# Illumina/canvas

Hardware: AMD Instinct MI355X
Metric: genome-bins/sec (bin+clean+partition) (higher is better)
Workload: dtype u8/int32 (bin), f32/f64 (clean, viterbi); 1 GPU; BASELINE configs[2]: whole-genome GRCh38 60x single sample, full bin+clean+partition HIP path on 1 MI355X per sample; bins_after_clean=4686240, bin_size=534, partition=PerSampleHMM, clean_flags=-g -s -r --local-sd-metric-file, segments=250, samples=1

## Files before the change

### canvas_amd/csrc/bin.hip

```cpp
#include "common.hpp"
#include <algorithm>
#include <thread>
#include <emmintrin.h>

#define TILE_SHIFT 12
#define TILE 4096

struct BinChrom {
    const uint8_t* bases;
    const uint8_t* hits;
    const uint64_t* mask;
    int64_t len;
    int64_t tileBase;
    int64_t ntiles;
};

__device__ __forceinline__ int find_chrom(const BinChrom* __restrict__ ch, int nchr, int64_t gtile) {
    int lo = 0, hi = nchr - 1;
    while (lo < hi) {
        int mid = (lo + hi + 1) >> 1;
        if (ch[mid].tileBase <= gtile) lo = mid; else hi = mid - 1;
    }
    return lo;
}
// ... 779 lines not shown
        ProfScope ps(ctx, "gcw_read_gc", false, sp);
        if (rg3) hipLaunchKernelGGL((k_read_gc3<RG3_HE, RG3_HO>), dim3((unsigned)std::min<int64_t>(gridRg, ntileAll)), dim3(256), ldsRg, sp, dRg, nchr, ntileAll, meanFrag, mean40, nWmax, hist);
        else for (int c = 0; c < nchr; c++) {
            const int64_t ntile = (h_len[c] + RG_T - 1) / RG_T;
            hipLaunchKernelGGL(k_read_gc2, dim3((unsigned)std::min<int64_t>(gridRg, ntile)), dim3(256), ldsRg, sp, d_bases[c], d_fraglen[c], d_hits[c], h_len[c], meanFrag, mean40, nWmax,
                               (uint8_t*)gch[c].readGc, hist);
        }
    }
    CANVAS_HIP_TRY(ctx, hipMemcpyAsync(ctx->side_pin, hist, (size_t)RG_REP_ALL * 202 * 8, hipMemcpyDeviceToHost, sp));
    CANVAS_HIP_TRY(ctx, hipEventRecord(ctx->side_ev2, sp));
    P.pending = true;
    if (!P.overlap) { rc0 = gcw_prepass_finish(ctx, P); if (rc0) return rc0; }
    return CANVAS_OK;
}

static int32_t bin_genome_impl(canvas_ctx* ctx, int32_t nchr, const uint8_t* const* d_bases, const uint64_t* const* d_mask,
                               const uint8_t* const* d_hits, const int16_t* const* d_fraglen, const int64_t* h_len, const uint8_t* h_is_auto, int32_t counts_per_bin, int32_t bin_size, int32_t mode,
                               int32_t* d_chr, int32_t* d_start, int32_t* d_stop, int32_t* d_gc, float* d_count, int64_t cap,
                               int32_t* h_bin_size_out, int64_t* h_nbins_per_chr, int64_t* h_nbins_total, cvx_bin_size_hook hook = nullptr, void* hookUser = nullptr,
                               const int64_t* h_pos0_packed = nullptr) {
    if (!ctx) return CANVAS_ERR_INVALID;
    const bool needRates = bin_size <= 0;
    const bool packed = h_pos0_packed != nullptr;
    if (nchr <= 0 || !d_bases || !d_mask || !d_hits || !h_len || (needRates && !hook && (!h_is_auto || counts_per_bin <= 0))) CANVAS_FAIL(ctx, CANVAS_ERR_INVALID, "canvas_bin_genome: bad arguments");
    const bool gcw = mode == CANVAS_MODE_GC_CONTENT_WEIGHTED;
    if (gcw && !d_fraglen) CANVAS_FAIL(ctx, CANVAS_ERR_INVALID, "GCContentWeighted mode needs the fragment-length arrays (canvas_bin_sample_gcweighted)");
    if (gcw && packed) CANVAS_FAIL(ctx, CANVAS_ERR_INVALID, "the packed planes serve Binary and TruncatedDynamicRange; GCContentWeighted reads the per-base arrays");
    if (mode != CANVAS_MODE_BINARY && mode != CANVAS_MODE_TRUNCATED_DYNAMIC_RANGE && !gcw) CANVAS_FAIL(ctx, CANVAS_ERR_INVALID, "unknown coverage mode");
    for (int c = 0; c < nchr; c++) if (h_len[c] <= 0 || h_len[c] > 0x7FFFFFFFll) CANVAS_FAIL(ctx, CANVAS_ERR_INVALID, "chromosome length must be in [1, 2^31)");
    CANVAS_HIP_TRY(ctx, hipSetDevice(ctx->device));
    BinPlan plan = make_plan(nchr, d_bases, d_mask, d_hits, h_len);
    GcwPre gp;
    if (gcw) { ctx->gcw_stats_dev = nullptr; ctx->gcw_total = 0; }
    if (gcw && ctx->up_active) {
        CANVAS_HIP_TRY(ctx, hipStreamSynchronize(ctx->copy)); ctx->up_active = false;
    }
    if (gcw) {
        for (int c = 0; c < nchr; c++) if (((uintptr_t)d_fraglen[c] | (uintptr_t)d_bases[c] | (uintptr_t)d_hits[c]) & 15) CANVAS_FAIL(ctx, CANVAS_ERR_INVALID, "GCContentWeighted mode: bases, hits and fragment lengths must be 16-byte aligned");
        int32_t rc0 = gcw_prepass_begin(ctx, nchr, d_bases, d_hits, d_fraglen, h_len, true, gp); if (rc0) return rc0;
    }
    const int64_t ub = cap;
    WsSizer sz;
    const size_t tabSlots = (size_t)nchr + ((size_t)nchr + sizeof(BinChrom) - 1) / sizeof(BinChrom);
    sz.take<BinChrom>(tabSlots); sz.take<unsigned long long>(nchr); sz.take<uint32_t>(plan.ntiles); sz.take<uint32_t>(plan.ntiles); sz.take<int32_t>(plan.ntiles);
    sz.take<ChromOut>(nchr); sz.take<long long>(nchr + 1); sz.take<uint32_t>(plan.ntiles); sz.take<uint32_t>(plan.ntiles);
    sz.take<int32_t>(ub + 1); sz.take<uint32_t>(ub + 1); sz.take<uint32_t>(ub + 1);
    bool streamed = ctx->up_active && (int)ctx->up_bases.size() == nchr && !gcw;
    for (int c = 0; streamed && c < nchr; c++) streamed = ctx->up_bases[c] == d_bases[c] && ctx->up_mask[c] == d_mask[c] && ctx->up_hits[c] == d_hits[c];
    if (ctx->up_active && !streamed) { CANVAS_HIP_TRY(ctx, hipStreamSynchronize(ctx->copy)); }
    ctx->up_active = false;
    const bool singleRead = packed || streamed || (needRates && !cvx_hook("CANVAS_BIN_TWO_PASS")) || cvx_hook("CANVAS_BIN_SINGLE_READ");
    const int nchunks = (int)((plan.ntiles + TS_CHUNK - 1) / TS_CHUNK);
    if (singleRead) { sz.take<uint32_t>(plan.ntiles * 64); sz.take<uint32_t>(plan.ntiles + 8); sz.take<TsPart>(nchunks + 1); sz.take<TsPart>(nchunks + 1); sz.take<unsigned long long>(nchr);
                      sz.take<TsPart>(nchr + 1); sz.take<ChromDev>(nchr); sz.take<uint4>(ub + 1); }
    int32_t rc = canvas_ws_reserve(ctx, sz.off + 4096); if (rc) return rc;
    const size_t oAuto = (size_t)nchr * sizeof(BinChrom), oOut = (oAuto + (size_t)nchr + 15) & ~size_t(15), oP0 = oOut + (size_t)nchr * sizeof(ChromOut), oBd = oP0 + (size_t)nchr * 8;
    rc = canvas_pin_reserve(ctx, oBd + sizeof(BinDev) + 64); if (rc) return rc;
    WsCarver ws(ctx->ws);
    BinChrom* dCh = ws.take<BinChrom>(tabSlots); unsigned long long* dPos0 = ws.take<unsigned long long>(nchr);
    uint32_t* tilePop = ws.take<uint32_t>(plan.ntiles); uint32_t* tileObs = ws.take<uint32_t>(plan.ntiles); int32_t* rankBase = ws.take<int32_t>(plan.ntiles);
    ChromOut* dOut = ws.take<ChromOut>(nchr); long long* binOffset = ws.take<long long>(nchr + 1);
    uint32_t* tileTotC = ws.take<uint32_t>(plan.ntiles); uint32_t* tileTotG = ws.take<uint32_t>(plan.ntiles);
    int32_t* stopTmp = ws.take<int32_t>(ub + 1); uint32_t* locC = ws.take<uint32_t>(ub + 1); uint32_t* locG = ws.take<uint32_t>(ub + 1);
    uint32_t* wordSum = singleRead ? ws.take<uint32_t>(plan.ntiles * 64) : nullptr;
    uint32_t* rankRaw = nullptr; TsPart* tsPart = nullptr; TsPart* tsPartEx = nullptr; unsigned long long* dPopBefore = nullptr; TsPart* chrPre = nullptr; ChromDev* chrDev = nullptr; uint4* binRec = nullptr; uint8_t* dIsAuto = (uint8_t*)(dCh + nchr);
    if (singleRead) { rankRaw = ws.take<uint32_t>(plan.ntiles + 8); tsPart = ws.take<TsPart>(nchunks + 1); tsPartEx = ws.take<TsPart>(nchunks + 1); dPopBefore = ws.take<unsigned long long>(nchr);
                      chrPre = ws.take<TsPart>(nchr + 1); chrDev = ws.take<ChromDev>(nchr); binRec = ws.take<uint4>(ub + 1); }
    if (singleRead && !ctx->bin_dev) {
        CANVAS_HIP_TRY(ctx, hipMalloc(&ctx->bin_dev, 256)); CANVAS_HIP_TRY(ctx, hipMemsetAsync(ctx->bin_dev, 0, 256, ctx->stream));
        CANVAS_HIP_TRY(ctx, hipEventCreateWithFlags(&ctx->bin_ev, hipEventDisableTiming));
    }
    uint32_t* dTick = (uint32_t*)ctx->bin_dev; BinDev* dBd = (BinDev*)((char*)ctx->bin_dev + 64);
    const int clampHits = mode == CANVAS_MODE_TRUNCATED_DYNAMIC_RANGE ? 1 : 0;
    const bool byVal = nchr <= BIN_BYVAL;
    if (byVal) {
        BinChromPack pack; memset(&pack, 0, sizeof pack);
        memcpy(pack.c, plan.chroms.data(), nchr * sizeof(BinChrom));
        for (int c = 0; c < nchr; c++) {
            pack.isAuto[c] = h_is_auto ? (h_is_auto[c] ? 1 : 0) : 0;
            if (packed) { if (h_pos0_packed[c] < 0 || h_pos0_packed[c] > h_len[c]) CANVAS_FAIL(ctx, CANVAS_ERR_INVALID, "canvas_bin_sample_packed: pos0 outside [0, len]"); pack.pos0[c] = (unsigned long long)h_pos0_packed[c]; }
        }
        hipLaunchKernelGGL(k_bin_begin, dim3(1), dim3(256), 0, ctx->stream, dCh, dIsAuto, pack, nchr, dPos0, packed ? 1 : 0);
    } else {
        memcpy(ctx->pin, plan.chroms.data(), nchr * sizeof(BinChrom));
        for (int c = 0; c < nchr; c++) ((uint8_t*)ctx->pin)[oAuto + c] = h_is_auto ? (h_is_auto[c] ? 1 : 0) : 0;
        CANVAS_HIP_TRY(ctx, hipMemcpyAsync(dCh, ctx->pin, oAuto + (size_t)nchr, hipMemcpyHostToDevice, ctx->stream));
    }
    ChromOut* hOut = (ChromOut*)((char*)ctx->pin + oOut);
    const unsigned pkGrid = (unsigned)((plan.ntiles + 4 * PK_TILES - 1) / (4 * PK_TILES));
    if (packed) {
        if (!byVal) {
            unsigned long long* hp0 = (unsigned long long*)((char*)ctx->pin + oP0);
            for (int c = 0; c < nchr; c++) {
                if (h_pos0_packed[c] < 0 || h_pos0_packed[c] > h_len[c]) CANVAS_FAIL(ctx, CANVAS_ERR_INVALID, "canvas_bin_sample_packed: pos0 outside [0, len]");
                hp0[c] = (unsigned long long)h_pos0_packed[c];
            }
            CANVAS_HIP_TRY(ctx, hipMemcpyAsync(dPos0, hp0, (size_t)nchr * 8, hipMemcpyHostToDevice, ctx->stream));
        }
        if (streamed) {
            for (int c = 0; c < nchr; c++) {
                const BinChrom& C = plan.chroms[c];
                CANVAS_HIP_TRY(ctx, hipStreamWaitEvent(ctx->stream, ctx->up_ev[c], 0));
                ProfScope ps(ctx, "bin_summary_packed_streamed", true);
                hipLaunchKernelGGL(k_tile_summary_packed, dim3((unsigned)((C.ntiles + 4 * PK_TILES - 1) / (4 * PK_TILES))), dim3(256), 0, ctx->stream, dCh, nchr, C.tileBase + C.ntiles, dPos0,
                                   clampHits, needRates ? 1 : 0, wordSum, tilePop, tileObs, tileTotC, tileTotG, C.tileBase);
            }
        } else {
            ProfScope ps(ctx, "bin_summary_packed", true);
            hipLaunchKernelGGL(k_tile_summary_packed, dim3(pkGrid), dim3(256), 0, ctx->stream, dCh, nchr, plan.ntiles, dPos0, clampHits, needRates ? 1 : 0,
                               wordSum, tilePop, tileObs, tileTotC, tileTotG, (int64_t)0);
        }
    } else {
    if (!byVal) hipLaunchKernelGGL(k_init_pos0, dim3((nchr + 63) / 64), dim3(64), 0, ctx->stream, dCh, nchr, dPos0);
    if (streamed) {
        for (int c = 0; c < nchr; c++) {
            const BinChrom& C = plan.chroms[c];
            CANVAS_HIP_TRY(ctx, hipStreamWaitEvent(ctx->stream, ctx->up_ev[c], 0));
            hipLaunchKernelGGL(k_find_pos0, dim3(64, 1), dim3(256), 0, ctx->stream, dCh, dPos0, c);
            ProfScope ps(ctx, "bin_summary_streamed", true);
            hipLaunchKernelGGL(k_tile_summary, dim3((unsigned)((C.ntiles + 3) / 4)), dim3(256), 0, ctx->stream, dCh, nchr, C.tileBase + C.ntiles, dPos0, clampHits, needRates ? 1 : 0,
                               wordSum, tilePop, tileObs, tileTotC, tileTotG, C.tileBase);
            hipLaunchKernelGGL(k_tile_summary_edges, dim3(2), dim3(64), 0, ctx->stream, dCh, nchr, dPos0, clampHits, needRates ? 1 : 0, wordSum, tilePop, tileObs, tileTotC, tileTotG, c);
        }
    } else hipLaunchKernelGGL(k_find_pos0, dim3(64, nchr), dim3(256), 0, ctx->stream, dCh, dPos0, 0);
    if (streamed) {
    } else if (singleRead) {
        ProfScope ps(ctx, "bin_summary", true);
        hipLaunchKernelGGL(k_tile_summary, dim3((unsigned)((plan.ntiles + 3) / 4)), dim3(256), 0, ctx->stream, dCh, nchr, plan.ntiles, dPos0, clampHits, needRates ? 1 : 0,
                           wordSum, tilePop, tileObs, tileTotC, tileTotG, (int64_t)0);
    } else {
        ProfScope ps(ctx, "bin_tile_stats", true);
        hipLaunchKernelGGL(k_tile_stats, dim3((unsigned)((plan.ntiles + 3) / 4)), dim3(256), 0, ctx->stream, dCh, nchr, plan.ntiles, needRates ? 1 : 0, tilePop, tileObs);
    }
    if (singleRead && !streamed) hipLaunchKernelGGL(k_tile_summary_edges, dim3(2 * nchr), dim3(64), 0, ctx->stream, dCh, nchr, dPos0, clampHits, needRates ? 1 : 0, wordSum, tilePop, tileObs, tileTotC, tileTotG, 0);
    }
    int64_t total = 0;
    if (singleRead) {
        const int binSizeArg = !needRates ? bin_size : (hook ? -1 : 0);
        const uint32_t* obsArr = needRates ? tileObs : (const uint32_t*)nullptr;
        unsigned* hBdSeq = (unsigned*)((char*)ctx->pin + oBd + sizeof(BinDev));
        const unsigned bdSeq = hook ? 0u : cvx_mail_arm(ctx, hBdSeq);
        hipLaunchKernelGGL(k_tscan_reduce, dim3((unsigned)(nchunks + nchr)), dim3(TS_T), 0, ctx->stream, dCh, nchr, dPos0, packed ? 1 : 0, plan.ntiles, nchunks, tilePop, obsArr, tileTotC, tileTotG,
                           tsPart, tsPartEx, dPopBefore, dTick);
        hipLaunchKernelGGL(k_tscan_apply, dim3((unsigned)nchunks), dim3(TS_T), 0, ctx->stream, dCh, nchr, plan.ntiles, nchunks, tilePop, obsArr, tileTotC, tileTotG, rankRaw, tsPartEx, dPopBefore, chrPre,
                           dIsAuto, counts_per_bin, binSizeArg, (long long)cap, dOut, chrDev, binOffset, dBd, dTick + 1, hook ? (ChromOut*)nullptr : hOut, hook ? (BinDev*)nullptr : (BinDev*)((char*)ctx->pin + oBd),
                           hBdSeq, bdSeq);
        auto launch_close_resolve = [&]() {
            { ProfScope ps(ctx, "bin_close");
              hipLaunchKernelGGL(k_bin_close2, dim3((unsigned)((plan.ntiles + 4 * CLOSE_TILES - 1) / (4 * CLOSE_TILES))), dim3(256), 0, ctx->stream, dCh, chrDev, nchr, plan.ntiles, wordSum, rankRaw,
                                 tileTotC, tileTotG, binOffset, dBd, binRec, d_chr); }
            ProfScope ps(ctx, "bin_resolve");
            static const unsigned gridP = resident_grid((const void*)k_bin_resolve_fin<true>, 256, ctx->device), gridB = resident_grid((const void*)k_bin_resolve_fin<false>, 256, ctx->device);
            if (packed) hipLaunchKernelGGL((k_bin_resolve_fin<true>), dim3(gridP), dim3(256), 0, ctx->stream, dCh, chrDev, binOffset, dPos0, dBd, clampHits, binRec, d_start, d_stop, d_gc, d_count);
            else hipLaunchKernelGGL((k_bin_resolve_fin<false>), dim3(gridB), dim3(256), 0, ctx->stream, dCh, chrDev, binOffset, dPos0, dBd, clampHits, binRec, d_start, d_stop, d_gc, d_count);
        };
        auto host_totals = [&]() {
            total = 0;
            for (int c = 0; c < nchr; c++) { hOut[c].nbins = (hOut[c].pop - hOut[c].popBefore) / bin_size; if (h_nbins_per_chr) h_nbins_per_chr[c] = hOut[c].nbins; total += hOut[c].nbins; }
        };
        if (hook) {
            CANVAS_HIP_TRY(ctx, hipMemcpyAsync(hOut, dOut, nchr * sizeof(ChromOut), hipMemcpyDeviceToHost, ctx->stream));
            CANVAS_HIP_TRY(ctx, hipStreamSynchronize(ctx->stream));
            std::vector<long long> o(nchr), p(nchr), pb(nchr);
            for (int c = 0; c < nchr; c++) { o[c] = hOut[c].obs; p[c] = hOut[c].pop; pb[c] = hOut[c].popBefore; }
            int32_t rch = hook(hookUser, nchr, o.data(), p.data(), pb.data(), &bin_size); if (rch) return rch;
            if (bin_size <= 0) CANVAS_FAIL(ctx, CANVAS_ERR_INVALID, "derived bin size is not positive");
            if (h_bin_size_out) *h_bin_size_out = bin_size;
            host_totals();
            if (h_nbins_total) *h_nbins_total = total;
            if (total > cap) CANVAS_FAIL(ctx, CANVAS_ERR_CAPACITY, "canvas_bin_genome: output capacity too small (see canvas_bin_count_upper_bound)");
            if (total == 0) return CANVAS_OK;
            hipLaunchKernelGGL(k_bin_plan, dim3(1), dim3(TS_T), 0, ctx->stream, nchr, dOut, binOffset, dBd, bin_size, (long long)cap);
            launch_close_resolve();
        } else {
            BinDev* hBd = (BinDev*)((char*)ctx->pin + oBd);
            CANVAS_HIP_TRY(ctx, hipEventRecord(ctx->bin_ev, ctx->stream));
            launch_close_resolve();
            CANVAS_HIP_TRY(ctx, hipEventSynchronize(ctx->bin_ev));
            { int32_t rcm = cvx_mail_await(ctx, hBdSeq, bdSeq, "canvas_bin: bin size and totals"); if (rcm) return rcm; }
            if (needRates && (hBd->flags & (BD_BAD_RATE | BD_TOO_MANY))) {
                std::vector<double> rates;
                for (int c = 0; c < nchr; c++) if (h_is_auto[c]) rates.push_back((int)hOut[c].obs / (double)(int)hOut[c].pop);
                bin_size = canvas_bin_size_from_rates(rates.data(), (int32_t)rates.size(), counts_per_bin);
                if (bin_size <= 0) CANVAS_FAIL(ctx, CANVAS_ERR_INVALID, "derived bin size is not positive");
                host_totals();
                if (total <= cap && total > 0) { hipLaunchKernelGGL(k_bin_plan, dim3(1), dim3(TS_T), 0, ctx->stream, nchr, dOut, binOffset, dBd, bin_size, (long long)cap); launch_close_resolve(); }
            } else {
                if (needRates && (hBd->flags & BD_NO_AUTOSOME)) CANVAS_FAIL(ctx, CANVAS_ERR_INVALID, "no autosome to derive the bin size from");
                bin_size = hBd->binSize;
                if (bin_size <= 0) CANVAS_FAIL(ctx, CANVAS_ERR_INVALID, "derived bin size is not positive");
                total = hBd->total;
                for (int c = 0; c < nchr; c++) if (h_nbins_per_chr) h_nbins_per_chr[c] = hOut[c].nbins;
            }
            if (h_bin_size_out) *h_bin_size_out = bin_size;
            if (h_nbins_total) *h_nbins_total = total;
            if (total > cap) CANVAS_FAIL(ctx, CANVAS_ERR_CAPACITY, "canvas_bin_genome: output capacity too small (see canvas_bin_count_upper_bound)");
            if (total == 0) return CANVAS_OK;
        }
    } else {
    if (needRates) {
        hipLaunchKernelGGL(k_scan_tiles, dim3(nchr), dim3(1024), 0, ctx->stream, dCh, dPos0, tilePop, tileObs, 1, 0, rankBase, dOut, packed ? 1 : 0);
        CANVAS_HIP_TRY(ctx, hipMemcpyAsync(hOut, dOut, nchr * sizeof(ChromOut), hipMemcpyDeviceToHost, ctx->stream));
        CANVAS_HIP_TRY(ctx, hipStreamSynchronize(ctx->stream));
        if (hook) {
            std::vector<long long> o(nchr), p(nchr), pb(nchr);
            for (int c = 0; c < nchr; c++) { o[c] = hOut[c].obs; p[c] = hOut[c].pop; pb[c] = hOut[c].popBefore; }
            int32_t rch = hook(hookUser, nchr, o.data(), p.data(), pb.data(), &bin_size); if (rch) return rch;
// ... 440 lines not shown
```

### canvas_amd/csrc/bin_tail.hpp

```cpp
#pragma once

struct BinDev {
    int32_t binSize;
    int32_t run;
    unsigned long long binMagic;
    long long total;
    int32_t flags;
    int32_t nAuto;
};
#define BD_NO_AUTOSOME 1
#define BD_BAD_RATE 2
#define BD_TOO_MANY 4
#define BD_CAPACITY 8
struct ChromDev { uint32_t rank0, c0, g0, pad; };
struct TsPart { uint32_t pop, obs, c, g; };

#define TS_T 1024
#define TS_ITEMS 8
#define TS_CHUNK (TS_T * TS_ITEMS)
#define BD_MAX_AUTO 2048

template <class T> __device__ __forceinline__ void ts_publish(T* p, T v) { __hip_atomic_store(p, v, __ATOMIC_RELAXED, __HIP_MEMORY_SCOPE_AGENT); }
__device__ __forceinline__ bool ts_arrive_last(uint32_t* tick, uint32_t expected, int* sFlag) {
    asm volatile("s_waitcnt vmcnt(0)" ::: "memory");
// ... 177 lines not shown
            const int item = (int)(rel % TS_ITEMS);
            TsPart o = {0, 0, 0, 0};
#pragma unroll
            for (int i = 0; i < TS_ITEMS; i++) if (i == item) { o.pop = rp[i]; o.obs = ro[i]; o.c = rc[i]; o.g = rg[i]; }
            ts_publish(&chrPre[c].pop, o.pop); ts_publish(&chrPre[c].obs, o.obs); ts_publish(&chrPre[c].c, o.c); ts_publish(&chrPre[c].g, o.g);
        }
    }
    if (!ts_arrive_last(tick, gridDim.x, &sLast)) return;
    const TsPart grand = partEx[nchunks];
    if (tid == 0) { sN = 0; sFlags = 0; sBinSize = binSizeArg > 0 ? binSizeArg : 0; }
    __syncthreads();
    {
        const int per = (nchr + TS_T - 1) / TS_T;
        const int cA = tid * per < nchr ? tid * per : nchr, cB = cA + per < nchr ? cA + per : nchr;
        for (int c = cA; c < cB; c++) {
            const TsPart a = chrPre[c], e = c + 1 < nchr ? chrPre[c + 1] : grand;
            const unsigned long long pb = popBefore[c];
            ChromOut o; o.pop = (long long)(uint32_t)(e.pop - a.pop); o.obs = (long long)(uint32_t)(e.obs - a.obs); o.nbins = 0; o.popBefore = (long long)pb;
            dOut[c] = o;
            ChromDev d; d.rank0 = a.pop + (uint32_t)pb; d.c0 = a.c; d.g0 = a.g; d.pad = 0;
            chrDev[c] = d;
            if (binSizeArg == 0 && isAuto[c]) {
                if (o.pop <= 0) atomicOr(&sFlags, BD_BAD_RATE);
                const int slot = atomicAdd(&sN, 1);
                if (slot < BD_MAX_AUTO) sRate[slot] = (double)(int)o.obs / (double)(int)o.pop;
            }
        }
    }
    __syncthreads();
    if (binSizeArg == 0) {
        const int n = sN;
        if (n == 0) { if (tid == 0) sFlags |= BD_NO_AUTOSOME; }
        else if (n > BD_MAX_AUTO) { if (tid == 0) sFlags |= BD_TOO_MANY; }
        else if (!(sFlags & BD_BAD_RATE)) {
            for (int i = tid; i < n; i += TS_T) {
                const double r = sRate[i]; int rank = 0;
                for (int j = 0; j < n; j++) { const double q = sRate[j]; rank += (q < r || (q == r && j < i)) ? 1 : 0; }
                sSorted[rank] = r;
            }
            __syncthreads();
            if (tid == 0) {
                const double med = (n % 2) ? sSorted[n / 2] : (sSorted[n / 2 - 1] + sSorted[n / 2]) / 2;
                const double q = (double)countsPerBin / med;
                sBinSize = (q >= 1.0 && q < 2147483648.0) ? (int)q : 0;
            }
        }
        __syncthreads();
    }
    if (binSizeArg < 0) return;
    __syncthreads();
    plan_offsets(nchr, dOut, dOut, binOffset, bd, sBinSize, cap, sFlags, sN, sh16, hostOut, hostBd, hostSeq, seq);
}

__global__ void __launch_bounds__(256) k_bin_close2(const BinChrom* __restrict__ ch, const ChromDev* __restrict__ chrDev, int nchr, int64_t ntilesTotal, const uint32_t* __restrict__ S,
                                                    const uint32_t* __restrict__ rankRaw, const uint32_t* __restrict__ tileExC, const uint32_t* __restrict__ tileExG,
                                                    const long long* __restrict__ binOffset, const BinDev* __restrict__ bd,
                                                    uint4* __restrict__ binRec, int32_t* __restrict__ oChr) {
    const int64_t gtile0 = ((int64_t)blockIdx.x * 4 + __builtin_amdgcn_readfirstlane((int)(threadIdx.x >> 6))) * CLOSE_TILES;
    if (gtile0 >= ntilesTotal) return;
    if (!bd->run) return;
    const int binSize = bd->binSize; const unsigned long long binMagic = bd->binMagic;
    const int l = lane_id();
    uint32_t sv[CLOSE_TILES], rk[CLOSE_TILES], tc[CLOSE_TILES], tg[CLOSE_TILES];
#pragma unroll
    for (int t = 0; t < CLOSE_TILES; t++) {
        const bool in = gtile0 + t < ntilesTotal;
        sv[t] = in ? S[(gtile0 + t) * 64 + l] : 0u;
        rk[t] = in ? rankRaw[gtile0 + t] : 0u;
        tc[t] = in ? tileExC[gtile0 + t] : 0u;
        tg[t] = in ? tileExG[gtile0 + t] : 0u;
    }
    int c = find_chrom(ch, nchr, gtile0);
    int64_t tileBase = ch[c].tileBase, tileEnd = tileBase + ch[c].ntiles;
    long long boff = binOffset[c];
    uint32_t rank0 = chrDev[c].rank0;
#pragma unroll
    for (int t = 0; t < CLOSE_TILES; t++) {
        const int64_t gtile = gtile0 + t;
        if (gtile >= ntilesTotal) break;
        while (gtile >= tileEnd) { c++; tileBase = ch[c].tileBase; tileEnd = tileBase + ch[c].ntiles; boff = binOffset[c]; rank0 = chrDev[c].rank0; }
        const uint32_t s = sv[t];
        const uint32_t pop = SUM_POP(s);
        const uint32_t pg = pop | (SUM_GC(s) << 16), cl = SUM_HITS(s);
        const uint32_t pgInc = wave_inclusive_scan_u32(pg), cInc = wave_inclusive_scan_u32(cl);
        const int32_t r = (int32_t)(rk[t] - rank0) + (int32_t)((pgInc - pg) & 0xFFFFu);
        if (pop > 0 && r + (int32_t)pop >= binSize) {
            const uint32_t gEx = tg[t] + ((pgInc - pg) >> 16), cEx = tc[t] + (cInc - cl);
            const int64_t wstart = ((gtile - tileBase) << TILE_SHIFT) + (int64_t)l * 64;
            const int32_t rr = r < 0 ? 0 : r;
            uint32_t q = binMagic ? (uint32_t)__umul64hi((unsigned long long)(uint32_t)rr, binMagic) : (uint32_t)rr;
            uint32_t nextB = (q + 1u) * (uint32_t)binSize;
            for (; (int64_t)nextB - r <= (int64_t)pop && (int64_t)nextB - r >= 1; q++) {
                const long long bin = boff + (long long)q;
                binRec[bin] = make_uint4((uint32_t)(wstart + ((int64_t)nextB - r - 1)), cEx, gEx, (uint32_t)c);
                oChr[bin] = c;
                nextB += (uint32_t)binSize;
            }
        }
    }
}

template <class T> __device__ __forceinline__ uint4 gload_uint4_nt(gptr<T> p) { const canvas_u32x4 v = __builtin_nontemporal_load(reinterpret_cast<gptr<const canvas_u32x4>>(p)); return make_uint4(v.x, v.y, v.z, v.w); }
template <class T> __device__ __forceinline__ ulonglong2 gload_ulonglong2_nt(gptr<T> p) { const canvas_u64x2 v = __builtin_nontemporal_load(reinterpret_cast<gptr<const canvas_u64x2>>(p)); return make_ulonglong2(v.x, v.y); }

__device__ __forceinline__ uint32_t kth_set_bit(uint64_t m, uint32_t kk) {
    uint32_t pos = 0, cnt;
    cnt = __popc((uint32_t)m);           if (kk > cnt) { kk -= cnt; pos += 32; m >>= 32; }
    cnt = __popc((uint32_t)m & 0xFFFFu); if (kk > cnt) { kk -= cnt; pos += 16; m >>= 16; }
    cnt = __popc((uint32_t)m & 0xFFu);   if (kk > cnt) { kk -= cnt; pos += 8; m >>= 8; }
    cnt = __popc((uint32_t)m & 0xFu);    if (kk > cnt) { kk -= cnt; pos += 4; m >>= 4; }
    cnt = __popc((uint32_t)m & 0x3u);    if (kk > cnt) { kk -= cnt; pos += 2; m >>= 2; }
    cnt = (uint32_t)m & 1u;              if (kk > cnt) { pos += 1; }
    return pos;
}
template <bool PACKED>
__global__ void __launch_bounds__(256) k_bin_resolve_fin(const BinChrom* __restrict__ ch, const ChromDev* __restrict__ chrDev, const long long* __restrict__ binOffset,
                                                         const unsigned long long* __restrict__ pos0, const BinDev* __restrict__ bd, int clampHits,
                                                         const uint4* __restrict__ binRec,
                                                         int32_t* __restrict__ oStart, int32_t* __restrict__ oStop, int32_t* __restrict__ oGc, float* __restrict__ oCount) {
    constexpr int LANES = PACKED ? 1 : 4, SLOTS = 256 / LANES, RF_NEW = SLOTS - 1;
    __shared__ int32_t sStop[SLOTS], sChr[SLOTS]; __shared__ uint32_t sC[SLOTS], sG[SLOTS];
    if (!bd->run) return;
    const long long total = bd->total;
    const long long ngroups = (total + RF_NEW - 1) / RF_NEW;
    const int slot = threadIdx.x / LANES, sub = threadIdx.x % LANES;
    for (long long g = blockIdx.x; g < ngroups; g += gridDim.x) {
        const long long i = g * RF_NEW - 1 + slot;
        const bool live = i >= 0 && i < total;
        int32_t stop = 0; uint32_t aC = 0, aG = 0, hc = 0, hg = 0; int c = 0;
        if (live) {
            const uint4 R = binRec[i];
            const int32_t r = (int32_t)R.x;
            c = (int)R.w;
            aC = R.y; aG = R.z;
            const int64_t p0c = (int64_t)pos0[c];
            const int64_t wstart = (int64_t)(r & ~63);
            uint32_t kk = (uint32_t)(r & 63) + 1u;
            uint64_t mw, valid = ~0ull;
            if (PACKED) {
                const int64_t w = wstart >> 6;
                const gptr<const ulonglong2> hp = reinterpret_cast<gptr<const ulonglong2>>(as_global(ch[c].hits));
                const ulonglong2 rr = gload_ulonglong2_nt(reinterpret_cast<gptr<const ulonglong2>>(as_global(ch[c].bases)) + w);
                const ulonglong2 ha = gload_ulonglong2_nt(hp + 2 * w), hb = gload_ulonglong2_nt(hp + 2 * w + 1);
                valid = pk_valid(wstart, p0c);
                mw = rr.x;
                const uint32_t pos = kth_set_bit(mw, kk);
                const unsigned long long head = valid & ((2ull << pos) - 1ull);
                unsigned long long b0 = ha.x, b1 = ha.y, b2 = hb.x; const unsigned long long b3 = hb.y;
                if (clampHits) pk_clamp10(b0, b1, b2, b3);
                hc = pk_masked_sum(b0, b1, b2, b3, mw & head);
                hg = (uint32_t)__popcll(rr.y & head);
                stop = (int32_t)(wstart + pos + 1);
            } else {
                const gptr<const uint8_t> bases = as_global(ch[c].bases), hits = as_global(ch[c].hits);
                const int64_t len = ch[c].len;
                const int64_t cstart = wstart + 16 * sub;
                mw = __builtin_nontemporal_load(as_global(ch[c].mask) + (wstart >> 6));
                uint32_t wb[4] = {0, 0, 0, 0}, wh[4] = {0, 0, 0, 0};
                if (cstart + 16 <= len) {
                    const uint4 bb = gload_uint4_nt(bases + cstart), hh = gload_uint4_nt(hits + cstart);
                    wb[0] = bb.x; wb[1] = bb.y; wb[2] = bb.z; wb[3] = bb.w; wh[0] = hh.x; wh[1] = hh.y; wh[2] = hh.z; wh[3] = hh.w;
                } else {
                    for (int j = 0; j < 16; j++) { const int64_t pi = cstart + j; if (pi < len) { wb[j >> 2] |= (uint32_t)bases[pi] << (8 * (j & 3)); wh[j >> 2] |= (uint32_t)hits[pi] << (8 * (j & 3)); } }
                }
                if (len - wstart < 64) { valid = (~0ull) >> (64 - (len - wstart)); mw &= valid; }
                if (wstart < p0c) valid = (p0c - wstart >= 64) ? 0ull : (valid & ((~0ull) << (p0c - wstart)));
                const uint32_t pos = kth_set_bit(mw, kk);
                const uint64_t head = valid & ((2ull << pos) - 1ull);
                const uint32_t head16 = (uint32_t)(head >> (16 * sub)) & 0xFFFFu, mVal16 = (uint32_t)(mw >> (16 * sub)) & head16;
                uint32_t gc16 = 0;
#pragma unroll
                for (int q = 0; q < 4; q++) {
                    gc16 |= marks_to_bits4(gc_marks4(wb[q])) << (4 * q);
                    const uint32_t h = clampHits ? clamp10_bytes(wh[q]) : wh[q];
                    hc = sum_bytes(h & expand4(mVal16 >> (4 * q)), hc);
                }
                hg = __popc(gc16 & head16);
                stop = (int32_t)(wstart + pos + 1);
            }
        }
        if (!PACKED) {
            hc += __shfl_xor(hc, 1, 64); hg += __shfl_xor(hg, 1, 64);
            hc += __shfl_xor(hc, 2, 64); hg += __shfl_xor(hg, 2, 64);
        }
        if (sub == 0) { sStop[slot] = stop; sC[slot] = aC + hc; sG[slot] = aG + hg; sChr[slot] = c; }
        __syncthreads();
        {
            const int s2 = threadIdx.x;
            const long long i2 = g * RF_NEW - 1 + s2;
            if (s2 > 0 && s2 < SLOTS && i2 < total) {
                const int c2 = sChr[s2];
                const bool first = i2 == binOffset[c2];
                const int32_t stop2 = sStop[s2];
                const int32_t start = first ? (int32_t)pos0[c2] : sStop[s2 - 1];
                const uint32_t pC = first ? chrDev[c2].c0 : sC[s2 - 1], pG = first ? chrDev[c2].g0 : sG[s2 - 1];
                const uint32_t count = sC[s2] - pC, gcCount = sG[s2] - pG;
                float gcf = 100.0f * (float)(int32_t)gcCount;
                gcf = gcf / (float)(stop2 - start);
                oStart[i2] = start; oStop[i2] = stop2; oGc[i2] = (int32_t)gcf; oCount[i2] = (float)(int32_t)count;
            }
        }
        __syncthreads();
    }
}
```

Baseline: 2.041 billion bins/s.

## Fuse bin close and resolve kernels into a single per-wave tail kernel

Replaces the two-kernel sequence (k_bin_close2 writing per-bin boundary records to a global binRec array, then k_bin_resolve_fin reading them back) with one k_bin_tail kernel. Each wave stages its tiles' summaries in LDS, emits bin boundary events into a per-wave LDS buffer and flushes them in batches of 64, computing start/stop/gc/count directly. To seed the first bin it searches backwards through rankRaw for the tile holding the preceding boundary. This removes a global round-trip of a uint4 per bin and one kernel launch, at the cost of more LDS, extra boundary searches per wave, and more complex wave-serial flush logic.

```diff
diff --git a/canvas_amd/csrc/bin.hip b/canvas_amd/csrc/bin.hip
--- a/canvas_amd/csrc/bin.hip
+++ b/canvas_amd/csrc/bin.hip
@@ -855,7 +855,7 @@
     const bool singleRead = packed || streamed || (needRates && !cvx_hook("CANVAS_BIN_TWO_PASS")) || cvx_hook("CANVAS_BIN_SINGLE_READ");
     const int nchunks = (int)((plan.ntiles + TS_CHUNK - 1) / TS_CHUNK);
     if (singleRead) { sz.take<uint32_t>(plan.ntiles * 64); sz.take<uint32_t>(plan.ntiles + 8); sz.take<TsPart>(nchunks + 1); sz.take<TsPart>(nchunks + 1); sz.take<unsigned long long>(nchr);
-                      sz.take<TsPart>(nchr + 1); sz.take<ChromDev>(nchr); sz.take<uint4>(ub + 1); }
+                      sz.take<TsPart>(nchr + 1); sz.take<ChromDev>(nchr); }
     int32_t rc = canvas_ws_reserve(ctx, sz.off + 4096); if (rc) return rc;
     const size_t oAuto = (size_t)nchr * sizeof(BinChrom), oOut = (oAuto + (size_t)nchr + 15) & ~size_t(15), oP0 = oOut + (size_t)nchr * sizeof(ChromOut), oBd = oP0 + (size_t)nchr * 8;
     rc = canvas_pin_reserve(ctx, oBd + sizeof(BinDev) + 64); if (rc) return rc;
@@ -866,9 +866,9 @@
     uint32_t* tileTotC = ws.take<uint32_t>(plan.ntiles); uint32_t* tileTotG = ws.take<uint32_t>(plan.ntiles);
     int32_t* stopTmp = ws.take<int32_t>(ub + 1); uint32_t* locC = ws.take<uint32_t>(ub + 1); uint32_t* locG = ws.take<uint32_t>(ub + 1);
     uint32_t* wordSum = singleRead ? ws.take<uint32_t>(plan.ntiles * 64) : nullptr;
-    uint32_t* rankRaw = nullptr; TsPart* tsPart = nullptr; TsPart* tsPartEx = nullptr; unsigned long long* dPopBefore = nullptr; TsPart* chrPre = nullptr; ChromDev* chrDev = nullptr; uint4* binRec = nullptr; uint8_t* dIsAuto = (uint8_t*)(dCh + nchr);
+    uint32_t* rankRaw = nullptr; TsPart* tsPart = nullptr; TsPart* tsPartEx = nullptr; unsigned long long* dPopBefore = nullptr; TsPart* chrPre = nullptr; ChromDev* chrDev = nullptr; uint8_t* dIsAuto = (uint8_t*)(dCh + nchr);
     if (singleRead) { rankRaw = ws.take<uint32_t>(plan.ntiles + 8); tsPart = ws.take<TsPart>(nchunks + 1); tsPartEx = ws.take<TsPart>(nchunks + 1); dPopBefore = ws.take<unsigned long long>(nchr);
-                      chrPre = ws.take<TsPart>(nchr + 1); chrDev = ws.take<ChromDev>(nchr); binRec = ws.take<uint4>(ub + 1); }
+                      chrPre = ws.take<TsPart>(nchr + 1); chrDev = ws.take<ChromDev>(nchr); }
     if (singleRead && !ctx->bin_dev) {
         CANVAS_HIP_TRY(ctx, hipMalloc(&ctx->bin_dev, 256)); CANVAS_HIP_TRY(ctx, hipMemsetAsync(ctx->bin_dev, 0, 256, ctx->stream));
         CANVAS_HIP_TRY(ctx, hipEventCreateWithFlags(&ctx->bin_ev, hipEventDisableTiming));
@@ -949,13 +949,12 @@
                            dIsAuto, counts_per_bin, binSizeArg, (long long)cap, dOut, chrDev, binOffset, dBd, dTick + 1, hook ? (ChromOut*)nullptr : hOut, hook ? (BinDev*)nullptr : (BinDev*)((char*)ctx->pin + oBd),
                            hBdSeq, bdSeq);
         auto launch_close_resolve = [&]() {
-            { ProfScope ps(ctx, "bin_close");
-              hipLaunchKernelGGL(k_bin_close2, dim3((unsigned)((plan.ntiles + 4 * CLOSE_TILES - 1) / (4 * CLOSE_TILES))), dim3(256), 0, ctx->stream, dCh, chrDev, nchr, plan.ntiles, wordSum, rankRaw,
-                                 tileTotC, tileTotG, binOffset, dBd, binRec, d_chr); }
             ProfScope ps(ctx, "bin_resolve");
-            static const unsigned gridP = resident_grid((const void*)k_bin_resolve_fin<true>, 256, ctx->device), gridB = resident_grid((const void*)k_bin_resolve_fin<false>, 256, ctx->device);
-            if (packed) hipLaunchKernelGGL((k_bin_resolve_fin<true>), dim3(gridP), dim3(256), 0, ctx->stream, dCh, chrDev, binOffset, dPos0, dBd, clampHits, binRec, d_start, d_stop, d_gc, d_count);
-            else hipLaunchKernelGGL((k_bin_resolve_fin<false>), dim3(gridB), dim3(256), 0, ctx->stream, dCh, chrDev, binOffset, dPos0, dBd, clampHits, binRec, d_start, d_stop, d_gc, d_count);
+            const unsigned grid = (unsigned)((plan.ntiles + 4 * BT_TILES - 1) / (4 * BT_TILES));
+            if (packed) hipLaunchKernelGGL((k_bin_tail<true>), dim3(grid), dim3(256), 0, ctx->stream, dCh, chrDev, nchr, plan.ntiles, wordSum, rankRaw, tileTotC, tileTotG, binOffset, dPos0, dBd, clampHits,
+                                           d_chr, d_start, d_stop, d_gc, d_count);
+            else hipLaunchKernelGGL((k_bin_tail<false>), dim3(grid), dim3(256), 0, ctx->stream, dCh, chrDev, nchr, plan.ntiles, wordSum, rankRaw, tileTotC, tileTotG, binOffset, dPos0, dBd, clampHits,
+                                    d_chr, d_start, d_stop, d_gc, d_count);
         };
         auto host_totals = [&]() {
             total = 0;
diff --git a/canvas_amd/csrc/bin_tail.hpp b/canvas_amd/csrc/bin_tail.hpp
--- a/canvas_amd/csrc/bin_tail.hpp
+++ b/canvas_amd/csrc/bin_tail.hpp
@@ -253,54 +253,8 @@
     plan_offsets(nchr, dOut, dOut, binOffset, bd, sBinSize, cap, sFlags, sN, sh16, hostOut, hostBd, hostSeq, seq);
 }
 
-__global__ void __launch_bounds__(256) k_bin_close2(const BinChrom* __restrict__ ch, const ChromDev* __restrict__ chrDev, int nchr, int64_t ntilesTotal, const uint32_t* __restrict__ S,
-                                                    const uint32_t* __restrict__ rankRaw, const uint32_t* __restrict__ tileExC, const uint32_t* __restrict__ tileExG,
-                                                    const long long* __restrict__ binOffset, const BinDev* __restrict__ bd,
-                                                    uint4* __restrict__ binRec, int32_t* __restrict__ oChr) {
-    const int64_t gtile0 = ((int64_t)blockIdx.x * 4 + __builtin_amdgcn_readfirstlane((int)(threadIdx.x >> 6))) * CLOSE_TILES;
-    if (gtile0 >= ntilesTotal) return;
-    if (!bd->run) return;
-    const int binSize = bd->binSize; const unsigned long long binMagic = bd->binMagic;
-    const int l = lane_id();
-    uint32_t sv[CLOSE_TILES], rk[CLOSE_TILES], tc[CLOSE_TILES], tg[CLOSE_TILES];
-#pragma unroll
-    for (int t = 0; t < CLOSE_TILES; t++) {
-        const bool in = gtile0 + t < ntilesTotal;
-        sv[t] = in ? S[(gtile0 + t) * 64 + l] : 0u;
-        rk[t] = in ? rankRaw[gtile0 + t] : 0u;
-        tc[t] = in ? tileExC[gtile0 + t] : 0u;
-        tg[t] = in ? tileExG[gtile0 + t] : 0u;
-    }
-    int c = find_chrom(ch, nchr, gtile0);
-    int64_t tileBase = ch[c].tileBase, tileEnd = tileBase + ch[c].ntiles;
-    long long boff = binOffset[c];
-    uint32_t rank0 = chrDev[c].rank0;
-#pragma unroll
-    for (int t = 0; t < CLOSE_TILES; t++) {
-        const int64_t gtile = gtile0 + t;
-        if (gtile >= ntilesTotal) break;
-        while (gtile >= tileEnd) { c++; tileBase = ch[c].tileBase; tileEnd = tileBase + ch[c].ntiles; boff = binOffset[c]; rank0 = chrDev[c].rank0; }
-        const uint32_t s = sv[t];
-        const uint32_t pop = SUM_POP(s);
-        const uint32_t pg = pop | (SUM_GC(s) << 16), cl = SUM_HITS(s);
-        const uint32_t pgInc = wave_inclusive_scan_u32(pg), cInc = wave_inclusive_scan_u32(cl);
-        const int32_t r = (int32_t)(rk[t] - rank0) + (int32_t)((pgInc - pg) & 0xFFFFu);
-        if (pop > 0 && r + (int32_t)pop >= binSize) {
-            const uint32_t gEx = tg[t] + ((pgInc - pg) >> 16), cEx = tc[t] + (cInc - cl);
-            const int64_t wstart = ((gtile - tileBase) << TILE_SHIFT) + (int64_t)l * 64;
-            const int32_t rr = r < 0 ? 0 : r;
-            uint32_t q = binMagic ? (uint32_t)__umul64hi((unsigned long long)(uint32_t)rr, binMagic) : (uint32_t)rr;
-            uint32_t nextB = (q + 1u) * (uint32_t)binSize;
-            for (; (int64_t)nextB - r <= (int64_t)pop && (int64_t)nextB - r >= 1; q++) {
-                const long long bin = boff + (long long)q;
-                binRec[bin] = make_uint4((uint32_t)(wstart + ((int64_t)nextB - r - 1)), cEx, gEx, (uint32_t)c);
-                oChr[bin] = c;
-                nextB += (uint32_t)binSize;
-            }
-        }
-    }
-}
-
+#define BT_TILES 8
+#define BT_SLOTS 64
 template <class T> __device__ __forceinline__ uint4 gload_uint4_nt(gptr<T> p) { const canvas_u32x4 v = __builtin_nontemporal_load(reinterpret_cast<gptr<const canvas_u32x4>>(p)); return make_uint4(v.x, v.y, v.z, v.w); }
 template <class T> __device__ __forceinline__ ulonglong2 gload_ulonglong2_nt(gptr<T> p) { const canvas_u64x2 v = __builtin_nontemporal_load(reinterpret_cast<gptr<const canvas_u64x2>>(p)); return make_ulonglong2(v.x, v.y); }
 
@@ -314,93 +268,189 @@
     cnt = (uint32_t)m & 1u;              if (kk > cnt) { pos += 1; }
     return pos;
 }
+__device__ __forceinline__ void wave_lds_sync() { __builtin_amdgcn_fence(__ATOMIC_RELEASE, "wavefront"); __builtin_amdgcn_wave_barrier(); __builtin_amdgcn_fence(__ATOMIC_ACQUIRE, "wavefront"); }
+__device__ __forceinline__ uint32_t bt_div(uint32_t x, unsigned long long binMagic) { return binMagic ? (uint32_t)__umul64hi((unsigned long long)x, binMagic) : x; }
+
 template <bool PACKED>
-__global__ void __launch_bounds__(256) k_bin_resolve_fin(const BinChrom* __restrict__ ch, const ChromDev* __restrict__ chrDev, const long long* __restrict__ binOffset,
-                                                         const unsigned long long* __restrict__ pos0, const BinDev* __restrict__ bd, int clampHits,
-                                                         const uint4* __restrict__ binRec,
-                                                         int32_t* __restrict__ oStart, int32_t* __restrict__ oStop, int32_t* __restrict__ oGc, float* __restrict__ oCount) {
-    constexpr int LANES = PACKED ? 1 : 4, SLOTS = 256 / LANES, RF_NEW = SLOTS - 1;
-    __shared__ int32_t sStop[SLOTS], sChr[SLOTS]; __shared__ uint32_t sC[SLOTS], sG[SLOTS];
+__global__ void __launch_bounds__(256) k_bin_tail(const BinChrom* __restrict__ ch, const ChromDev* __restrict__ chrDev, int nchr, int64_t ntilesTotal, const uint32_t* __restrict__ S,
+                                                  const uint32_t* __restrict__ rankRaw, const uint32_t* __restrict__ tileExC, const uint32_t* __restrict__ tileExG,
+                                                  const long long* __restrict__ binOffset, const unsigned long long* __restrict__ pos0, const BinDev* __restrict__ bd, int clampHits,
+                                                  int32_t* __restrict__ oChr, int32_t* __restrict__ oStart, int32_t* __restrict__ oStop, int32_t* __restrict__ oGc, float* __restrict__ oCount) {
+    constexpr int LANES = PACKED ? 1 : 4, PER = 64 / LANES, ROUNDS = BT_SLOTS / PER;
+    static_assert(BT_SLOTS == 64, "the last step of a flush takes one lane per slot");
+    __shared__ uint32_t sSumAll[4][BT_TILES * 64];
+    __shared__ uint4 sEvAll[4][BT_SLOTS];
+    __shared__ int32_t sStopAll[4][BT_SLOTS]; __shared__ uint32_t sCAll[4][BT_SLOTS], sGAll[4][BT_SLOTS];
+    const int w = __builtin_amdgcn_readfirstlane((int)(threadIdx.x >> 6)), l = lane_id();
+    const int64_t gtile0 = ((int64_t)blockIdx.x * 4 + w) * BT_TILES;
+    if (gtile0 >= ntilesTotal) return;
     if (!bd->run) return;
-    const long long total = bd->total;
-    const long long ngroups = (total + RF_NEW - 1) / RF_NEW;
-    const int slot = threadIdx.x / LANES, sub = threadIdx.x % LANES;
-    for (long long g = blockIdx.x; g < ngroups; g += gridDim.x) {
-        const long long i = g * RF_NEW - 1 + slot;
-        const bool live = i >= 0 && i < total;
-        int32_t stop = 0; uint32_t aC = 0, aG = 0, hc = 0, hg = 0; int c = 0;
-        if (live) {
-            const uint4 R = binRec[i];
-            const int32_t r = (int32_t)R.x;
-            c = (int)R.w;
-            aC = R.y; aG = R.z;
-            const int64_t p0c = (int64_t)pos0[c];
+    uint32_t* const sSum = sSumAll[w]; uint4* const sEv = sEvAll[w]; int32_t* const sStop = sStopAll[w]; uint32_t* const sC = sCAll[w]; uint32_t* const sG = sGAll[w];
+    const int binSize = bd->binSize; const unsigned long long binMagic = bd->binMagic; const long long total = bd->total;
+    const int nt = ntilesTotal - gtile0 < BT_TILES ? (int)(ntilesTotal - gtile0) : BT_TILES;
+#pragma unroll
+    for (int t = 0; t < BT_TILES; t++) sSum[t * 64 + l] = t < nt ? S[(gtile0 + t) * 64 + l] : 0u;
+    uint32_t rk = 0, tc = 0, tg = 0;
+    if (l < nt) { rk = rankRaw[gtile0 + l]; tc = tileExC[gtile0 + l]; tg = tileExG[gtile0 + l]; }
+    int c = find_chrom(ch, nchr, gtile0);
+    int64_t tileBase = ch[c].tileBase, tileEnd = tileBase + ch[c].ntiles;
+    long long boff = binOffset[c];
+    uint32_t rank0 = chrDev[c].rank0;
+    const int32_t r0 = (int32_t)((uint32_t)__builtin_amdgcn_readlane((int)rk, 0) - rank0);
+    const uint32_t nbBefore = r0 > 0 ? bt_div((uint32_t)r0, binMagic) : 0u;
+    const long long b0 = boff + (long long)nbBefore;
+    bool res0 = false;
+    if (nbBefore > 0u && (long long)nbBefore < binOffset[c + 1] - boff) {
+        const int32_t target = (int32_t)(nbBefore * (uint32_t)binSize);
+        if (l == 0) sEv[0] = make_uint4(0u, 0u, 0u, (uint32_t)c);
+        int64_t hi = gtile0, T = tileBase;
+        for (;;) {
+            const int64_t Tl = hi - 1 - l;
+            const bool below = Tl >= tileBase && (int32_t)(rankRaw[Tl] - rank0) < target;
+            const unsigned long long m = __ballot(below);
+            if (m) { T = hi - 1 - (int64_t)__builtin_ctzll(m); break; }
+            hi -= 64;
+            if (hi <= tileBase) break;
+        }
+        const uint32_t s = S[T * 64 + l];
+        const uint32_t pop = SUM_POP(s);
+        const uint32_t pg = pop | (SUM_GC(s) << 16), cl = SUM_HITS(s);
+        const uint32_t pgInc = wave_inclusive_scan_u32(pg), cInc = wave_inclusive_scan_u32(cl);
+        const int32_t r = (int32_t)(rankRaw[T] - rank0) + (int32_t)((pgInc - pg) & 0xFFFFu);
+        if (pop > 0 && r < target && target <= r + (int32_t)pop) {
+            const int64_t wstart = ((T - tileBase) << TILE_SHIFT) + (int64_t)l * 64;
+            sEv[0] = make_uint4((uint32_t)(wstart + ((int64_t)target - r - 1)), tileExC[T] + (cInc - cl), tileExG[T] + ((pgInc - pg) >> 16), (uint32_t)c);
+        }
+        res0 = true;
+    }
+    int base = 0, next = 0;
+    auto flush = [&](const int nslots) {
+        wave_lds_sync();
+        uint4 ev[ROUNDS]; bool live[ROUNDS];
+        uint64_t mw[ROUNDS]; int32_t p0c[ROUNDS], len[ROUNDS];
+        uint32_t da[ROUNDS][4], db[ROUNDS][4], dc[ROUNDS][4];
+        const int sub = l % LANES;
+#pragma unroll
+        for (int rd = 0; rd < ROUNDS; rd++) {
+            const int s = rd * PER + l / LANES;
+            live[rd] = s < nslots && (s > 0 || res0);
+            ev[rd] = make_uint4(0, 0, 0, 0); mw[rd] = 0; p0c[rd] = 0; len[rd] = 0;
+#pragma unroll
+            for (int j = 0; j < 4; j++) { da[rd][j] = 0; db[rd][j] = 0; dc[rd][j] = 0; }
+            if (live[rd]) {
+                ev[rd] = sEv[s];
+                const int cc = (int)ev[rd].w;
+                const int64_t wstart = (int64_t)((int32_t)ev[rd].x & ~63);
+                p0c[rd] = (int32_t)pos0[cc];
+                if (PACKED) {
+                    const int64_t wd = wstart >> 6;
+                    const gptr<const ulonglong2> hp = reinterpret_cast<gptr<const ulonglong2>>(as_global(ch[cc].hits));
+                    const uint4 rr = gload_uint4_nt(reinterpret_cast<gptr<const ulonglong2>>(as_global(ch[cc].bases)) + wd);
+                    const uint4 ha = gload_uint4_nt(hp + 2 * wd), hb = gload_uint4_nt(hp + 2 * wd + 1);
+                    da[rd][0] = rr.x; da[rd][1] = rr.y; da[rd][2] = rr.z; da[rd][3] = rr.w;
+                    db[rd][0] = ha.x; db[rd][1] = ha.y; db[rd][2] = ha.z; db[rd][3] = ha.w;
+                    dc[rd][0] = hb.x; dc[rd][1] = hb.y; dc[rd][2] = hb.z; dc[rd][3] = hb.w;
+                } else {
+                    const gptr<const uint8_t> bases = as_global(ch[cc].bases), hits = as_global(ch[cc].hits);
+                    const int64_t len64 = ch[cc].len;
+                    len[rd] = (int32_t)len64;
+                    const int64_t cstart = wstart + 16 * sub;
+                    mw[rd] = __builtin_nontemporal_load(as_global(ch[cc].mask) + (wstart >> 6));
+                    if (cstart + 16 <= len64) {
+                        const uint4 bb = gload_uint4_nt(bases + cstart), hh = gload_uint4_nt(hits + cstart);
+                        da[rd][0] = bb.x; da[rd][1] = bb.y; da[rd][2] = bb.z; da[rd][3] = bb.w; db[rd][0] = hh.x; db[rd][1] = hh.y; db[rd][2] = hh.z; db[rd][3] = hh.w;
+                    } else {
+                        for (int j = 0; j < 16; j++) { const int64_t pi = cstart + j; if (pi < len64) { da[rd][j >> 2] |= (uint32_t)bases[pi] << (8 * (j & 3)); db[rd][j >> 2] |= (uint32_t)hits[pi] << (8 * (j & 3)); } }
+                    }
+                }
+            }
+        }
+#pragma unroll
+        for (int rd = 0; rd < ROUNDS; rd++) {
+            const int s = rd * PER + l / LANES;
+            const int32_t r = (int32_t)ev[rd].x;
             const int64_t wstart = (int64_t)(r & ~63);
-            uint32_t kk = (uint32_t)(r & 63) + 1u;
-            uint64_t mw, valid = ~0ull;
+            const uint32_t kk = (uint32_t)(r & 63) + 1u;
+            int32_t stop = 0; uint32_t hc = 0, hg = 0;
             if (PACKED) {
-                const int64_t w = wstart >> 6;
-                const gptr<const ulonglong2> hp = reinterpret_cast<gptr<const ulonglong2>>(as_global(ch[c].hits));
-                const ulonglong2 rr = gload_ulonglong2_nt(reinterpret_cast<gptr<const ulonglong2>>(as_global(ch[c].bases)) + w);
-                const ulonglong2 ha = gload_ulonglong2_nt(hp + 2 * w), hb = gload_ulonglong2_nt(hp + 2 * w + 1);
-                valid = pk_valid(wstart, p0c);
-                mw = rr.x;
-                const uint32_t pos = kth_set_bit(mw, kk);
+                const uint64_t m = (uint64_t)da[rd][0] | ((uint64_t)da[rd][1] << 32), gcw = (uint64_t)da[rd][2] | ((uint64_t)da[rd][3] << 32);
+                const uint64_t valid = pk_valid(wstart, (int64_t)p0c[rd]);
+                const uint32_t pos = kth_set_bit(m, kk);
                 const unsigned long long head = valid & ((2ull << pos) - 1ull);
-                unsigned long long b0 = ha.x, b1 = ha.y, b2 = hb.x; const unsigned long long b3 = hb.y;
-                if (clampHits) pk_clamp10(b0, b1, b2, b3);
-                hc = pk_masked_sum(b0, b1, b2, b3, mw & head);
-                hg = (uint32_t)__popcll(rr.y & head);
+                unsigned long long h0 = (uint64_t)db[rd][0] | ((uint64_t)db[rd][1] << 32), h1 = (uint64_t)db[rd][2] | ((uint64_t)db[rd][3] << 32);
+                unsigned long long h2 = (uint64_t)dc[rd][0] | ((uint64_t)dc[rd][1] << 32); const unsigned long long h3 = (uint64_t)dc[rd][2] | ((uint64_t)dc[rd][3] << 32);
+                if (clampHits) pk_clamp10(h0, h1, h2, h3);
+                hc = pk_masked_sum(h0, h1, h2, h3, m & head);
+                hg = (uint32_t)__popcll(gcw & head);
                 stop = (int32_t)(wstart + pos + 1);
             } else {
-                const gptr<const uint8_t> bases = as_global(ch[c].bases), hits = as_global(ch[c].hits);
-                const int64_t len = ch[c].len;
-                const int64_t cstart = wstart + 16 * sub;
-                mw = __builtin_nontemporal_load(as_global(ch[c].mask) + (wstart >> 6));
-                uint32_t wb[4] = {0, 0, 0, 0}, wh[4] = {0, 0, 0, 0};
-                if (cstart + 16 <= len) {
-                    const uint4 bb = gload_uint4_nt(bases + cstart), hh = gload_uint4_nt(hits + cstart);
-                    wb[0] = bb.x; wb[1] = bb.y; wb[2] = bb.z; wb[3] = bb.w; wh[0] = hh.x; wh[1] = hh.y; wh[2] = hh.z; wh[3] = hh.w;
-                } else {
-                    for (int j = 0; j < 16; j++) { const int64_t pi = cstart + j; if (pi < len) { wb[j >> 2] |= (uint32_t)bases[pi] << (8 * (j & 3)); wh[j >> 2] |= (uint32_t)hits[pi] << (8 * (j & 3)); } }
-                }
-                if (len - wstart < 64) { valid = (~0ull) >> (64 - (len - wstart)); mw &= valid; }
-                if (wstart < p0c) valid = (p0c - wstart >= 64) ? 0ull : (valid & ((~0ull) << (p0c - wstart)));
-                const uint32_t pos = kth_set_bit(mw, kk);
+                uint64_t m = mw[rd], valid = ~0ull;
+                const int64_t len64 = (int64_t)len[rd], p064 = (int64_t)p0c[rd];
+                if (live[rd] && len64 - wstart < 64) { valid = (~0ull) >> (64 - (len64 - wstart)); m &= valid; }
+                if (wstart < p064) valid = (p064 - wstart >= 64) ? 0ull : (valid & ((~0ull) << (p064 - wstart)));
+                const uint32_t pos = kth_set_bit(m, kk);
                 const uint64_t head = valid & ((2ull << pos) - 1ull);
-                const uint32_t head16 = (uint32_t)(head >> (16 * sub)) & 0xFFFFu, mVal16 = (uint32_t)(mw >> (16 * sub)) & head16;
+                const uint32_t head16 = (uint32_t)(head >> (16 * sub)) & 0xFFFFu, mVal16 = (uint32_t)(m >> (16 * sub)) & head16;
                 uint32_t gc16 = 0;
 #pragma unroll
                 for (int q = 0; q < 4; q++) {
-                    gc16 |= marks_to_bits4(gc_marks4(wb[q])) << (4 * q);
-                    const uint32_t h = clampHits ? clamp10_bytes(wh[q]) : wh[q];
+                    gc16 |= marks_to_bits4(gc_marks4(da[rd][q])) << (4 * q);
+                    const uint32_t h = clampHits ? clamp10_bytes(db[rd][q]) : db[rd][q];
                     hc = sum_bytes(h & expand4(mVal16 >> (4 * q)), hc);
                 }
                 hg = __popc(gc16 & head16);
                 stop = (int32_t)(wstart + pos + 1);
-            }
-        }
-        if (!PACKED) {
-            hc += __shfl_xor(hc, 1, 64); hg += __shfl_xor(hg, 1, 64);
-            hc += __shfl_xor(hc, 2, 64); hg += __shfl_xor(hg, 2, 64);
-        }
-        if (sub == 0) { sStop[slot] = stop; sC[slot] = aC + hc; sG[slot] = aG + hg; sChr[slot] = c; }
-        __syncthreads();
+                hc += __shfl_xor(hc, 1, 64); hg += __shfl_xor(hg, 1, 64);
+                hc += __shfl_xor(hc, 2, 64); hg += __shfl_xor(hg, 2, 64);
+            }
+            if (live[rd] && sub == 0) { sStop[s] = stop; sC[s] = ev[rd].y + hc; sG[s] = ev[rd].z + hg; }
+        }
+        wave_lds_sync();
         {
-            const int s2 = threadIdx.x;
-            const long long i2 = g * RF_NEW - 1 + s2;
-            if (s2 > 0 && s2 < SLOTS && i2 < total) {
-                const int c2 = sChr[s2];
+            const long long i2 = b0 + (long long)(base + l - 1);
+            if (l > 0 && l < nslots && i2 < total) {
+                const int c2 = (int)sEv[l].w;
                 const bool first = i2 == binOffset[c2];
-                const int32_t stop2 = sStop[s2];
-                const int32_t start = first ? (int32_t)pos0[c2] : sStop[s2 - 1];
-                const uint32_t pC = first ? chrDev[c2].c0 : sC[s2 - 1], pG = first ? chrDev[c2].g0 : sG[s2 - 1];
-                const uint32_t count = sC[s2] - pC, gcCount = sG[s2] - pG;
+                const int32_t stop2 = sStop[l];
+                const int32_t start = first ? (int32_t)pos0[c2] : sStop[l - 1];
+                const uint32_t pC = first ? chrDev[c2].c0 : sC[l - 1], pG = first ? chrDev[c2].g0 : sG[l - 1];
+                const uint32_t count = sC[l] - pC, gcCount = sG[l] - pG;
                 float gcf = 100.0f * (float)(int32_t)gcCount;
                 gcf = gcf / (float)(stop2 - start);
-                oStart[i2] = start; oStop[i2] = stop2; oGc[i2] = (int32_t)gcf; oCount[i2] = (float)(int32_t)count;
-            }
-        }
-        __syncthreads();
-    }
-}
+                oChr[i2] = c2; oStart[i2] = start; oStop[i2] = stop2; oGc[i2] = (int32_t)gcf; oCount[i2] = (float)(int32_t)count;
+            }
+        }
+        wave_lds_sync();
+        if (l == 0) { sStop[0] = sStop[nslots - 1]; sC[0] = sC[nslots - 1]; sG[0] = sG[nslots - 1]; }
+        res0 = false;
+        wave_lds_sync();
+    };
+    for (int t = 0; t < nt; t++) {
+        const int64_t gtile = gtile0 + t;
+        while (gtile >= tileEnd) { c++; tileBase = ch[c].tileBase; tileEnd = tileBase + ch[c].ntiles; boff = binOffset[c]; rank0 = chrDev[c].rank0; }
+        const uint32_t s = sSum[t * 64 + l];
+        const uint32_t pop = SUM_POP(s);
+        const uint32_t pg = pop | (SUM_GC(s) << 16), cl = SUM_HITS(s);
+        const uint32_t pgInc = wave_inclusive_scan_u32(pg), cInc = wave_inclusive_scan_u32(cl);
+        const int32_t r = (int32_t)((uint32_t)__builtin_amdgcn_readlane((int)rk, t) - rank0) + (int32_t)((pgInc - pg) & 0xFFFFu);
+        const uint32_t gEx = (uint32_t)__builtin_amdgcn_readlane((int)tg, t) + ((pgInc - pg) >> 16), cEx = (uint32_t)__builtin_amdgcn_readlane((int)tc, t) + (cInc - cl);
+        const int64_t wstart = ((gtile - tileBase) << TILE_SHIFT) + (int64_t)l * 64;
+        uint32_t q = 0, n = 0;
+        if (pop > 0 && r + (int32_t)pop >= binSize) { q = bt_div((uint32_t)(r < 0 ? 0 : r), binMagic); n = bt_div((uint32_t)(r + (int32_t)pop), binMagic) - q; }
+        const int fb = (int)(boff - b0) + (int)q;
+        const int thi = next + __builtin_amdgcn_readfirstlane((int)wave_reduce_add_u32(n));
+        int done = next;
+        do {
+            const int wEnd = base + (BT_SLOTS - 1);
+            const int lim = thi < wEnd ? thi : wEnd;
+            const int bA = fb > done ? fb : done, bB = fb + (int)n < lim ? fb + (int)n : lim;
+            for (int b = bA; b < bB; b++) {
+                const uint32_t nextB = (q + (uint32_t)(b - fb) + 1u) * (uint32_t)binSize;
+                sEv[b - base + 1] = make_uint4((uint32_t)(wstart + ((int64_t)nextB - r - 1)), cEx, gEx, (uint32_t)c);
+            }
+            done = lim;
+            if (done == wEnd || (t == nt - 1 && done == thi && done > base)) { flush(done - base + 1); base = done; }
+        } while (done < thi);
+        next = thi;
+    }
+}
```

Result: slower. 1.928 billion bins/s (-5.5%).
